# aaakulchyk/replicann

Hardware: AMD Instinct MI355X
Metric: train-step samples/sec (whole node), GPT-2-small DDP at 1/2/4/8 MI355X (higher is better)
Workload: dtype bf16; 1 GPU; model=gpt2-small, global_batch=64, micro_batch_per_gpu=64, seq_len=1024, parallelism=dp1, optimizer=fused AdamW (fp32 master) + grad-norm clip, comm_world=1, gemm_cu_reserve=0

## Files before the change

### csrc/include/gemm_pk.h

```cpp
#pragma once
#include <type_traits>

#include "gemm_impl.h"

namespace rn_gemm_detail {

constexpr int PK_HALF = 16384;
constexpr int PK_RING = 8 * PK_HALF;
constexpr int PK_LDS = PK_RING + 64;
constexpr int PK_CTR_STRIDE = 32;
constexpr int PK_SCHED_INTS = 10 * PK_CTR_STRIDE;

RN_DEV int swz_kcp(int r) { return (((r >> 3) & 3) << 1) | ((r >> 1) & 1); }
RN_DEV int swz_mnp(int k) { return ((k >> 1) & 1) | (((k >> 3) & 1) << 2); }

template <bool KC, bool PERM>
RN_DEV void pk_stage(const u32x4& rs, long ld, int mn_lim, int k_lim, char* lds, int wave, int lane, bool live) {
#pragma unroll
    for (int i = 0; i < 2; ++i) {
        const int ins = wave * 2 + i;
        uint32_t voff;
        if constexpr (KC) {
            const int r = ins * 8 + (lane >> 3);
            const int cg = (lane & 7) ^ (PERM ? swz_kcp(r) : swz_kc(r));
            const int k = cg * 8;
            const bool ok = live && (r < mn_lim) && (k < k_lim);
            voff = ok ? (uint32_t)(((long)r * ld + k) * 2) : 0xFFFFFFF0u;
        } else {
            const int sub = ins >> 3, within = ins & 7;
            const int r = within * 8 + (lane >> 3);
            const int cg = (lane & 7) ^ (PERM ? swz_mnp(r) : swz_mn(r));
            const int mn = sub * 64 + cg * 8;
            const bool ok = live && (r < k_lim) && (mn < mn_lim);
            voff = ok ? (uint32_t)(((long)r * ld + mn) * 2) : 0xFFFFFFF0u;
        }
        dma16(rs, voff, lds + ins * 1024);
    }
}

RN_DEV int swz_f8(int r) { return ((r >> 1) & 3) | (((r >> 4) & 1) << 2); }

RN_DEV s16x8 pk_frag8_mn(const char* lds, int col0, int s, int lane) {
    typedef int i32x2v __attribute__((ext_vector_type(2)));
    const int g = lane >> 4, ii = lane & 15, q = ii >> 1, pp = ii & 1;
    const int cb = col0 + 8 * pp;
    i32x2v v[2];
#pragma unroll
    for (int t = 0; t < 2; ++t) {
        const int row = s * 64 + 16 * g + 8 * t + q;
        const char* a = lds + row * 128 + (((cb >> 4) ^ swz_f8(row)) << 4) + (cb & 15);
        v[t] = __builtin_amdgcn_ds_read_tr8_b64_v2i32((__attribute__((address_space(3))) i32x2v*)a);
    }
    const i32x4 w = {v[0][0], v[0][1], v[1][0], v[1][1]};
    return __builtin_bit_cast(s16x8, w);
}

template <bool KC>
RN_DEV s16x8 pk_frag_a(const char* lds, int mnbase, int s, int lane) {
    return frag<KC>(lds, mnbase, s, lane);
}

template <bool KC>
RN_DEV s16x8 pk_frag_b(const char* lds, int colbase, int j, int s, int lane) {
    if constexpr (KC) {
        const int i = lane & 15;
        const int row = colbase + 8 * (i >> 2) + 4 * j + (i & 3);
        const int chunk = s * 4 + (lane >> 4);
        return *reinterpret_cast<const s16x8*>(lds + row * 128 + ((chunk ^ swz_kcp(row)) << 4));
    } else {
        const char* sub = lds + (colbase >> 6) * 8192;
        const int cl = colbase & 63;
        const int g = lane >> 4, i = lane & 15, q = i >> 2, p = i & 3;
        const int c = (cl >> 3) + p;
        const int half = j ^ (p & 1);
        const int k0 = s * 32 + 8 * g + q;
        const int k1 = k0 + 4;
        const char* a0 = sub + k0 * 128 + ((c ^ swz_mnp(k0)) << 4) + half * 8;
        const char* a1 = sub + k1 * 128 + ((c ^ swz_mnp(k1)) << 4) + half * 8;
        s16x4 v0 = __builtin_amdgcn_ds_read_tr16_b64_v4i16((__attribute__((address_space(3))) s16x4*)a0);
        s16x4 v1 = __builtin_amdgcn_ds_read_tr16_b64_v4i16((__attribute__((address_space(3))) s16x4*)a1);
        s16x8 r;
        r[0] = v0[0]; r[1] = v0[1]; r[2] = v0[2]; r[3] = v0[3];
        r[4] = v1[0]; r[5] = v1[1]; r[6] = v1[2]; r[7] = v1[3];
        return r;
    }
}

RN_DEV __amdgpu_buffer_rsrc_t pk_rsrc(const void* base, uint32_t bytes) {
    const uint64_t bp = (uint64_t)base;
    const uint32_t lo = __builtin_amdgcn_readfirstlane((uint32_t)bp);
    const uint32_t hi = __builtin_amdgcn_readfirstlane((uint32_t)(bp >> 32));
    return __builtin_amdgcn_make_buffer_rsrc((void*)(((uint64_t)hi << 32) | lo), 0, bytes, 0x00020000);
}

RN_DEV u32x4 pk_rsrc_u(const void* base, uint32_t bytes) {
    const uint64_t bp = (uint64_t)base;
    u32x4 r;
    r[0] = __builtin_amdgcn_readfirstlane((uint32_t)bp);
    r[1] = __builtin_amdgcn_readfirstlane((uint32_t)(bp >> 32));
    r[2] = bytes;
    r[3] = 0x00020000u;
    return r;
}

#pragma clang diagnostic push
#pragma clang diagnostic ignored "-Winline-asm"
#if defined(RN_PK_ST_NT)
#define RN_PK_ST_POLICY "nt"
#elif defined(RN_PK_ST_SC)
#define RN_PK_ST_POLICY "sc0 sc1"
#else
#define RN_PK_ST_POLICY ""
#endif
RN_DEV void pk_st16(const u32x4 v, const u32x4& rs, uint32_t voff) {
    asm volatile("buffer_store_dwordx4 %0, %1, %2, 0 offen " RN_PK_ST_POLICY "\n\ts_nop 1" ::"v"(v), "v"(voff), "s"(rs) : "memory");
}
typedef unsigned u32x2v __attribute__((ext_vector_type(2)));
RN_DEV void pk_st8(const u32x2v v, const u32x4& rs, uint32_t voff) {
    asm volatile("buffer_store_dwordx2 %0, %1, %2, 0 offen\n\ts_nop 1" ::"v"(v), "v"(voff), "s"(rs) : "memory");
}
RN_DEV void pk_st16_nt(const u32x4 v, const u32x4& rs, uint32_t voff) {
    asm volatile("buffer_store_dwordx4 %0, %1, %2, 0 offen nt\n\ts_nop 1" ::"v"(v), "v"(voff), "s"(rs) : "memory");
}
#pragma clang diagnostic pop

RN_DEV uint32_t pk_pack2(float a, float b) {
    bf16x2 v = {(bf16)a, (bf16)b};
    return __builtin_bit_cast(uint32_t, v);
}
RN_DEV void pk_unpack8(const u32x4 u, float* f) {
    const uint32_t w[4] = {u.x, u.y, u.z, u.w};
#pragma unroll
    for (int d = 0; d < 4; ++d) {
        f[2 * d] = __builtin_bit_cast(float, w[d] << 16);
        f[2 * d + 1] = __builtin_bit_cast(float, w[d] & 0xFFFF0000u);
    }
}

template <int ACT, bool SPLIT, bool F32>
constexpr int pk_epi_stores() {
    return 16 * ((SPLIT || F32) ? 2 : 1) + (act_fwd(ACT) ? 16 : 0) + (act_bwd(ACT) ? 4 : 0);
}

RN_DEV i32x8 pk_cat8(const s16x8 a, const s16x8 b) {
    const i32x4 x = __builtin_bit_cast(i32x4, a), y = __builtin_bit_cast(i32x4, b);
    return (i32x8){x[0], x[1], x[2], x[3], y[0], y[1], y[2], y[3]};
}

#pragma clang diagnostic push
#pragma clang diagnostic ignored "-Winline-asm"
RN_DEV void pk_deq_issue(uint32_t& v, const int* ctr, bool live) {
    const u32x4 rs = pk_rsrc_u(ctr, ctr ? 4u : 0u);
    const uint32_t off = live ? 0u : 0xFFFFFFF0u;
    v = 1u;
    asm volatile("buffer_atomic_add %0, %1, %2, 0 offen sc0 ; rn_deq_issue" : "+v"(v) : "v"(off), "s"(rs) : "memory");
}
RN_DEV int pk_deq_take(uint32_t v) {
    asm volatile("; rn_deq_take %0" : "+v"(v));
    return (int)__builtin_amdgcn_readfirstlane(v);
}
#pragma clang diagnostic pop

template <bool AK, bool BKC, int ACT, bool SPLIT, bool F32, int DBG = 0, int FP8 = 0, bool DYN = false>
__global__ void __launch_bounds__(512, 1) gemm_pk(GemmArgs p) {
    static_assert(!FP8 || !(DBG & 8), "fp8: no DBG 8");
    static_assert(!FP8 || AK || (!BKC && SPLIT), "fp8 MN-contiguous A: weight gradient (both MN, split-K slabs) only");
    constexpr bool F8A_MN = FP8 && !AK;
    constexpr bool F8B_MN = FP8 && !BKC;
    constexpr bool F8MN = F8A_MN;
    static_assert(!F8B_MN || SPLIT || (ACT == ACT_NONE && !F32), "fp8 MN B, bf16 output: plain epilogue only");
    constexpr int S_EPI = (DBG & 64) ? 0 : pk_epi_stores<ACT, SPLIT, F32>() + ((F8B_MN && !SPLIT) ? 16 : 0);
    static_assert(!DYN || (!FP8 && DBG == 0), "dynamic schedule: bf16 production kernels only");
    constexpr int BM = 256, BN = 256;
    constexpr int WY = 6;
    static_assert(WY + 1 + S_EPI <= 63, "vmcnt range");
    extern __shared__ __attribute__((aligned(16))) char smem[];
    const int lane = threadIdx.x & 63;
    const int wave = __builtin_amdgcn_readfirstlane(threadIdx.x >> 6);
    const int wr = wave >> 2, wc = wave & 3;
    const int G = lane >> 4;
    const int tiles = p.tiles_m * p.tiles_n;
    const int items = tiles * p.split;
    const int grid = gridDim.x;
    const int bid = xcd_remap(blockIdx.x, grid);
    const int nk = p.k_per_split / BK;

    constexpr bool dyn = DYN;
    int* const ring = reinterpret_cast<int*>(smem + PK_RING);
    auto unit_of = [&](int s) -> int {
        if constexpr (!DYN) {
            const int u = bid + s * grid;
            return u < items ? u : -1;
        }
        return __builtin_amdgcn_readfirstlane(*(volatile int*)(ring + (s & 3)));
    };
    auto deq_map = [&](int q, int v) -> int {
        const int per = grid >> 3;
        const bool home = (grid & 7) == 0 && (per & (per - 1)) == 0;
        const int rh = home ? max(0, items / grid - 1) : 0;
        if (q < 8) {
            const int sh = 31 - __builtin_clz(per | 1);
            return (unsigned)v < (unsigned)(rh * per) ? (v >> sh) * grid + q * per + (v & (per - 1)) : -2;
        }
        return (unsigned)v < (unsigned)(items - rh * grid) ? rh * grid + v : -1;
    };

    float alpha = 1.f;
    if (p.alpha) alpha = *p.alpha;
    asm volatile("" ::"v"(alpha));

    auto item_coords = [&](int item, int& m0, int& n0, int& kb, int& ke, int& tm) {
        const int sid = item / tiles;
        int tn;
        group_tile(item - sid * tiles, p.tiles_m, p.tiles_n, tm, tn);
        m0 = tm * BM;
        n0 = tn * BN;
        kb = sid * p.k_per_split;
        ke = min(p.K, kb + p.k_per_split);
    };
    auto lane_mnk = [&](bool isA, int i, int& mn, int& k) {
        const int ins = wave * 2 + i;
        const bool kc = isA ? AK : BKC;
        if (kc) {
            mn = ins * 8 + (lane >> 3);
            k = ((lane & 7) ^ (isA ? swz_kc(mn) : swz_kcp(mn))) * 8;
        } else if (FP8) {
            k = ins * 8 + (lane >> 3);
            mn = ((lane & 7) ^ swz_f8(k)) * 16;
        } else {
            k = (ins & 7) * 8 + (lane >> 3);
            mn = (ins >> 3) * 64 + ((lane & 7) ^ (isA ? swz_mn(k) : swz_mnp(k))) * 8;
        }
    };
    uint32_t a_off[2], b_off[2];
#pragma unroll
    for (int i = 0; i < 2; ++i) {
        int mn, k;
        lane_mnk(true, i, mn, k);
        a_off[i] = (uint32_t)(F8A_MN ? (long)k * p.lda + mn : (AK ? (long)mn * p.lda + k : (long)k * p.lda + mn) * 2);
        lane_mnk(false, i, mn, k);
        b_off[i] = (uint32_t)(F8B_MN ? (long)k * p.ldb + mn : (BKC ? (long)mn * p.ldb + k : (long)k * p.ldb + mn) * 2);
    }
    const long a_step = AK ? (long)BK : (long)BK * p.lda, b_step = BKC ? (long)BK : (long)BK * p.ldb;
    const long a_half = AK ? 128L * p.lda : (F8A_MN ? 64L : 128L), b_half = BKC ? 128L * p.ldb : (F8B_MN ? 64L : 128L);
    const bf16* ca = p.A;
    const bf16* cb = p.B;
    int cml = 0, cnl = 0, ckl = 0, ckt = 0, ct = 0;
    int cu = -1, cs = 0;
    uint32_t intr = 0;
    auto cur_intr = [&]() {
        const bool kf = ckl >= BK;
        intr = kf ? ((cml >= 128 ? 1u : 0u) | (cnl >= 128 ? 2u : 0u) | (cnl >= 256 ? 4u : 0u) | (cml >= 256 ? 8u : 0u))
                  : 0u;
    };
    bool in_loop = false;
    auto cur_set = [&]() {
        int m0, n0, kb, ke, tm;
        item_coords(cu, m0, n0, kb, ke, tm);
        ca = AK ? p.A + (long)m0 * p.lda + kb : p.A + (long)kb * p.lda + (F8A_MN ? m0 / 2 : m0);
        cb = BKC ? p.B + (long)n0 * p.ldb + kb : p.B + (long)kb * p.ldb + (F8B_MN ? n0 / 2 : n0);
        cml = p.M - m0;
        cnl = p.N - n0;
        ckl = ke - kb;
        cur_intr();
    };
    auto cur_adv = [&]() {
        ++ct;
        if (cu < 0) return;
        if (++ckt < nk) {
            ca += a_step;
            cb += b_step;
            ckl -= BK;
            if (ckl < BK) intr = 0u;
            return;
        }
        ckt = 0;
        cu = unit_of(++cs);
        if (cu >= 0) {
            cur_set();
        } else {
            cml = cnl = ckl = 0;
            intr = 0u;
        }
    };
    const uint32_t lds0 = lds_addr(smem) + wave * 2048;
    auto issue_h = [&](auto hc) {
        constexpr int H = decltype(hc)::value;
        if constexpr (DBG & 1) {
            if (in_loop) return;
        }
        const uint32_t dst = lds0 + (uint32_t)(((ct & 1) * 4 + H) * PK_HALF);
        const bool isA = (H == 0 || H == 3);
        const bf16* base = isA ? (H == 3 ? ca + a_half : ca) : (H == 2 ? cb + b_half : cb);
        const int mnl = isA ? (H == 3 ? cml - 128 : cml) : (H == 2 ? cnl - 128 : cnl);
        const u32x4 rs = rsrc_sgpr(base);
        if constexpr (DBG & 16) {
            if (in_loop) {
#pragma unroll
                for (int i = 0; i < 2; ++i) dma16_at(rs, 0xFFFFFFF0u, dst + i * 1024);
                return;
            }
        }
        if (intr & (1u << H)) {
#pragma unroll
            for (int i = 0; i < 2; ++i) dma16_at(rs, isA ? a_off[i] : b_off[i], dst + i * 1024);
        } else {
#pragma unroll
            for (int i = 0; i < 2; ++i) {
                int mn, kk;
                lane_mnk(isA, i, mn, kk);
                const uint32_t o = isA ? a_off[i] : b_off[i];
                const bool f8mn = isA ? F8A_MN : F8B_MN;
                const bool kin = f8mn ? kk < 2 * ckl : kk < ckl;
                dma16_at(rs, (mn < mnl && kin) ? o : 0xFFFFFFF0u, dst + i * 1024);
            }
        }
    };
    using H0 = std::integral_constant<int, 0>;
    using H1 = std::integral_constant<int, 1>;
    using H2 = std::integral_constant<int, 2>;
    using H3 = std::integral_constant<int, 3>;

    f32x4 acc[2][2][4][2];
#pragma unroll
    for (int a = 0; a < 2; ++a)
#pragma unroll
        for (int b = 0; b < 2; ++b)
#pragma unroll
            for (int i = 0; i < 4; ++i)
#pragma unroll
                for (int j = 0; j < 2; ++j) acc[a][b][i][j] = (f32x4){0.f, 0.f, 0.f, 0.f};
    s16x8 Af[4][2], Bl[2][2], Br[2][2];
    auto frag_a = [&](const char* half, int mnbase, int s) -> s16x8 {
        if constexpr (F8A_MN) return pk_frag8_mn(half, mnbase, s, lane);
        else return pk_frag_a<AK>(half, mnbase, s, lane);
    };
    auto frag_b = [&](const char* half, int j, int s) -> s16x8 {
        if constexpr (F8B_MN) return pk_frag8_mn(half, wc * 32 + 16 * j, s, lane);
        else return pk_frag_b<BKC>(half, wc * 32, j, s, lane);
    };

    auto epilogue = [&](int m0, int n0, int tm, int sid) {
        const int mlim = p.M - m0, nlim = p.N - n0;
        const long ldc = SPLIT ? (long)p.N : p.ldc;
        constexpr int ES = (SPLIT || F32) ? 4 : 2;
        char* cbase = SPLIT ? (char*)(p.ws + ((long)sid * p.M + m0) * p.N + n0) : (char*)p.C + ((long)m0 * ldc + n0) * ES;
        const __amdgpu_buffer_rsrc_t crs = pk_rsrc(cbase, 0x7FFFFFF0u);
        const u32x4 crs_u = pk_rsrc_u(cbase, 0x7FFFFFF0u);
        auto off = [&](int mh, int i, int nh, int es, int dc = 0) -> uint32_t {
            const int r = mh * 128 + wr * 64 + i * 16 + (lane & 15);
            const int c = nh * 128 + wc * 32 + (F8B_MN ? 4 : 8) * G + dc;
            return (r < mlim && c < nlim) ? (uint32_t)(((long)r * ldc + c) * es) : 0xFFFFFFF0u;
        };
        float bias[2][8];
#pragma unroll
        for (int nh = 0; nh < 2; ++nh)
#pragma unroll
            for (int t = 0; t < 8; ++t) bias[nh][t] = 0.f;
        if (!SPLIT && !act_bwd(ACT) && p.bias) {
#pragma unroll
            for (int nh = 0; nh < 2; ++nh) {
                const int cb = n0 + nh * 128 + wc * 32;
                if (cb + 32 <= p.N) {
                    const __attribute__((address_space(4))) u32x4* bp =
                        (const __attribute__((address_space(4))) u32x4*)(p.bias + cb);
                    u32x4 b0 = bp[0], b1 = bp[1], b2 = bp[2], b3 = bp[3];
                    asm volatile("" : "+s"(b0), "+s"(b1), "+s"(b2), "+s"(b3));
                    const u32x4 bsel = G == 0 ? b0 : (G == 1 ? b1 : (G == 2 ? b2 : b3));
                    pk_unpack8(bsel, bias[nh]);
                } else if (cb + 8 * G < p.N) {
                    const u32x4 u = *reinterpret_cast<const u32x4*>(p.bias + cb + 8 * G);
                    pk_unpack8(u, bias[nh]);
                }
            }
        }
        const bf16* auxp = SPLIT ? nullptr
                                 : (act_bwd(ACT) ? p.pre : (p.res ? p.res : ((p.accumulate && !F32) ? (const bf16*)p.C : nullptr)));
        constexpr bool AUX2 = act_bwd(ACT) && !SPLIT && !F32;
        u32x4 aux[AUX2 ? 2 : 1][4][2];
        const __amdgpu_buffer_rsrc_t ars = pk_rsrc(auxp ? auxp + (long)m0 * p.ldc + n0 : nullptr, 0x7FFFFFF0u);
        const u32x4 prs = pk_rsrc_u(act_fwd(ACT) && p.pre ? (void*)(p.pre + (long)m0 * p.ldc + n0) : nullptr,
                                    act_fwd(ACT) && p.pre ? 0x7FFFFFF0u : 0u);
        float csum[2][8];
#pragma unroll
        for (int nh = 0; nh < 2; ++nh)
#pragma unroll
            for (int t = 0; t < 8; ++t) csum[nh][t] = 0.f;
#pragma unroll
        for (int mh = 0; mh < 2; ++mh) {
            if (auxp && (!AUX2 || mh == 0)) {
#pragma unroll
                for (int ah = 0; ah < (AUX2 ? 2 : 1); ++ah)
#pragma unroll
                for (int i = 0; i < 4; ++i)
#pragma unroll
                    for (int nh = 0; nh < 2; ++nh) {
#ifdef RN_PK_NO_AUX
                        aux[ah][i][nh] = (u32x4){0x3F803F80u, 0x3F803F80u, 0x3F803F80u, 0x3F803F80u};
#else
                        aux[ah][i][nh] = __builtin_amdgcn_raw_buffer_load_b128(ars, off(AUX2 ? ah : mh, i, nh, 2), 0, 0);
#endif
                    }
#ifndef RN_PK_NO_AUX
                __builtin_amdgcn_s_waitcnt(0x0F70);
#endif
            }
#pragma unroll
            for (int i = 0; i < 4; ++i)
#pragma unroll
                for (int nh = 0; nh < 2; ++nh) {
                    float v[8];
                    const bool swp = !BKC && !F8B_MN && (G & 1);
#pragma unroll
                    for (int c = 0; c < 8; ++c) {
                        const float x0 = acc[mh][nh][i][c >> 2][c & 3], x1 = acc[mh][nh][i][(c >> 2) ^ 1][c & 3];
                        v[c] = (swp ? x1 : x0) * alpha;
                    }
                    if constexpr (SPLIT) {
                        const uint32_t o = off(mh, i, nh, 4);
                        const uint32_t o2 = F8B_MN ? off(mh, i, nh, 4, 16) : (o == 0xFFFFFFF0u ? o : o + 16);
                        pk_st16((u32x4){__builtin_bit_cast(uint32_t, v[0]), __builtin_bit_cast(uint32_t, v[1]),
                                    __builtin_bit_cast(uint32_t, v[2]), __builtin_bit_cast(uint32_t, v[3])},
                            crs_u, o);
                        pk_st16((u32x4){__builtin_bit_cast(uint32_t, v[4]), __builtin_bit_cast(uint32_t, v[5]),
                                    __builtin_bit_cast(uint32_t, v[6]), __builtin_bit_cast(uint32_t, v[7])},
                            crs_u, o2);
                        continue;
                    }
#pragma unroll
                    for (int c = 0; c < 8; ++c) v[c] += bias[nh][c];
                    if constexpr (act_fwd(ACT)) {
                        const u32x4 pu = {pk_pack2(v[0], v[1]), pk_pack2(v[2], v[3]), pk_pack2(v[4], v[5]),
                                          pk_pack2(v[6], v[7])};
                        if constexpr (ACT == ACT_GELU_D) {
                            pk_unpack8(pu, v);
                            float d[8];
#pragma unroll
                            for (int c = 0; c < 8; ++c) v[c] = gelu_and_grad_f(v[c], d[c]);
                            const u32x4 du = {pk_pack2(d[0], d[1]), pk_pack2(d[2], d[3]), pk_pack2(d[4], d[5]),
                                              pk_pack2(d[6], d[7])};
                            pk_st16(du, prs, off(mh, i, nh, 2));
                        } else {
                            pk_st16(pu, prs, off(mh, i, nh, 2));
                            if (p.pre) pk_unpack8(pu, v);
#pragma unroll
                            for (int c = 0; c < 8; ++c) v[c] = act_f<ACT>(v[c]);
                        }
                    }
                    if (auxp) {
                        float ax[8];
                        pk_unpack8(aux[AUX2 ? mh : 0][i][nh], ax);
                        if constexpr (act_bwd(ACT)) {
#pragma unroll
                            for (int c = 0; c < 8; ++c) {
                                v[c] = (float)(bf16)v[c] * act_grad_f<ACT>(ax[c]);
                                csum[nh][c] += (float)(bf16)v[c];
                            }
                        } else {
#pragma unroll
                            for (int c = 0; c < 8; ++c) v[c] += ax[c];
                        }
                    }
                    const uint32_t o = off(mh, i, nh, ES);
                    if constexpr (F32) {
                        float c8[8] = {0.f, 0.f, 0.f, 0.f, 0.f, 0.f, 0.f, 0.f};
                        if (p.accumulate) {
                            const u32x4 c0 = __builtin_amdgcn_raw_buffer_load_b128(crs, o, 0, 0);
                            const u32x4 c1 = __builtin_amdgcn_raw_buffer_load_b128(crs, o == 0xFFFFFFF0u ? o : o + 16, 0, 0);
                            const uint32_t w[8] = {c0.x, c0.y, c0.z, c0.w, c1.x, c1.y, c1.z, c1.w};
#pragma unroll
                            for (int d = 0; d < 8; ++d) c8[d] = __builtin_bit_cast(float, w[d]);
                        }
#pragma unroll
                        for (int c = 0; c < 8; ++c) v[c] += c8[c];
                        pk_st16((u32x4){__builtin_bit_cast(uint32_t, v[0]), __builtin_bit_cast(uint32_t, v[1]),
                                    __builtin_bit_cast(uint32_t, v[2]), __builtin_bit_cast(uint32_t, v[3])},
                            crs_u, o);
                        pk_st16((u32x4){__builtin_bit_cast(uint32_t, v[4]), __builtin_bit_cast(uint32_t, v[5]),
                                    __builtin_bit_cast(uint32_t, v[6]), __builtin_bit_cast(uint32_t, v[7])},
                            crs_u, o == 0xFFFFFFF0u ? o : o + 16);
                    } else {
                        if (p.res && p.accumulate) {
                            float c8[8];
                            pk_unpack8(__builtin_amdgcn_raw_buffer_load_b128(crs, o, 0, 0), c8);
#pragma unroll
                            for (int c = 0; c < 8; ++c) v[c] += c8[c];
                        }
                        const u32x4 ou = {pk_pack2(v[0], v[1]), pk_pack2(v[2], v[3]), pk_pack2(v[4], v[5]),
                                          pk_pack2(v[6], v[7])};
                        if constexpr (DBG & 64) asm volatile("" ::"v"(ou));
                        else if constexpr (F8B_MN) {
                            pk_st8((u32x2v){ou.x, ou.y}, crs_u, o);
                            pk_st8((u32x2v){ou.z, ou.w}, crs_u, off(mh, i, nh, 2, 16));
                        } else if (p.st_nt & 1) pk_st16_nt(ou, crs_u, o);
                        else pk_st16(ou, crs_u, (DBG & 32) ? 0xFFFFFFF0u : o);
                    }
                }
        }
        if constexpr (act_bwd(ACT)) {
#pragma unroll
            for (int nh = 0; nh < 2; ++nh)
#pragma unroll
                for (int c = 0; c < 8; ++c) {
                    float s = csum[nh][c];
                    s += __shfl_xor(s, 1, 64);
                    s += __shfl_xor(s, 2, 64);
                    s += __shfl_xor(s, 4, 64);
                    s += __shfl_xor(s, 8, 64);
                    csum[nh][c] = s;
                }
            float* cpb = p.colpart ? p.colpart + ((long)tm * 2 + wr) * p.N + n0 : nullptr;
            const u32x4 cprs = pk_rsrc_u(cpb, cpb ? 0x7FFFFFF0u : 0u);
#pragma unroll
            for (int nh = 0; nh < 2; ++nh) {
                const int c = nh * 128 + wc * 32 + 8 * G;
                const uint32_t o = ((lane & 15) == 0 && c < nlim) ? (uint32_t)(c * 4) : 0xFFFFFFF0u;
                pk_st16((u32x4){__builtin_bit_cast(uint32_t, csum[nh][0]), __builtin_bit_cast(uint32_t, csum[nh][1]),
                            __builtin_bit_cast(uint32_t, csum[nh][2]), __builtin_bit_cast(uint32_t, csum[nh][3])},
                    cprs, o);
                pk_st16((u32x4){__builtin_bit_cast(uint32_t, csum[nh][4]), __builtin_bit_cast(uint32_t, csum[nh][5]),
                            __builtin_bit_cast(uint32_t, csum[nh][6]), __builtin_bit_cast(uint32_t, csum[nh][7])},
                    cprs, o == 0xFFFFFFF0u ? o : o + 16);
            }
        }
    };

    int deq = blockIdx.x & 7;
    uint32_t deq_v = 0u;

    if constexpr (DYN) {
        if (wave == 0 && lane == 0) {
            int q = blockIdx.x & 7;
            int u = deq_map(q, __hip_atomic_fetch_add(p.sched + q * PK_CTR_STRIDE, 1, __ATOMIC_RELAXED,
                                                      __HIP_MEMORY_SCOPE_AGENT));
            if (u == -2) {
                q = 8;
                u = deq_map(8, __hip_atomic_fetch_add(p.sched + 8 * PK_CTR_STRIDE, 1, __ATOMIC_RELAXED,
                                                      __HIP_MEMORY_SCOPE_AGENT));
            }
            ring[0] = u;
            ring[1] = q | (u < 0 ? 64 : 0);
        }
        __syncthreads();
        deq = __builtin_amdgcn_readfirstlane(ring[1]);
    }
    int c_s = 0;
    int c_u = unit_of(0);
    cu = c_u;
    if (cu >= 0) {
        cur_set();
        issue_h(H0{});
        issue_h(H1{});
        issue_h(H2{});
        issue_h(H3{});
        cur_adv();
        issue_h(H0{});
        issue_h(H1{});
    }
    vm_wait<8>();
    asm volatile("s_barrier" ::: "memory");
    if (wr == 1) asm volatile("s_barrier" ::: "memory");
    in_loop = true;
    __builtin_amdgcn_sched_barrier(0);

    int c_m0 = 0, c_n0 = 0, c_kb = 0, c_ke = 0, c_tm = 0, c_sid = 0, c_kt = 0;
    if (c_u >= 0) {
        item_coords(c_u, c_m0, c_n0, c_kb, c_ke, c_tm);
        c_sid = c_u / tiles;
    }
    int since_epi = 4;

    auto phase_wait = [&](auto xw) {
        if constexpr (DBG & 2) return;
        constexpr bool XW = decltype(xw)::value;
        if (since_epi < 4) {
            if (DYN && XW && wave == 0) vm_wait<WY + 1 + S_EPI>();
            else vm_wait<WY + S_EPI>();
        } else {
            if (DYN && XW && wave == 0) vm_wait<WY + 1>();
            else vm_wait<WY>();
        }
        ++since_epi;
    };
    auto deq_step = [&]() {
        if (DYN && wave == 0) {
            if (deq & 32) {
                const int u = deq_map(deq & 15, pk_deq_take(deq_v));
                if (u == -2) {
                    deq = (deq & 64) | 8 | 16;
                } else {
                    if (lane == 0) *(volatile int*)(ring + ((c_s + 1) & 3)) = u;
                    deq = (deq & ~32) | (u < 0 ? 64 : 0);
                }
            }
            const bool want = (deq & 16) != 0;
            pk_deq_issue(deq_v, p.sched + (deq & 15) * PK_CTR_STRIDE, lane == 0 && want);
            deq = (deq & ~48) | (want ? 32 : 0);
        }
    };
    auto sync_mma_begin = [&]() {
        __builtin_amdgcn_sched_barrier(0);
        asm volatile("s_barrier\n\ts_waitcnt lgkmcnt(0)" ::: "memory");
        __builtin_amdgcn_sched_barrier(0);
        __builtin_amdgcn_s_setprio(1);
    };
    auto sync_mma_end = [&]() {
        __builtin_amdgcn_s_setprio(0);
        __builtin_amdgcn_sched_barrier(0);
        asm volatile("s_barrier" ::: "memory");
        __builtin_amdgcn_sched_barrier(0);
    };
#define RN_PK_MMA(MH, NH, BF)                                                                          \
    if constexpr (FP8) {                                                                               \
        _Pragma("unroll") for (int i_ = 0; i_ < 4; ++i_)                                             \
        _Pragma("unroll") for (int j_ = 0; j_ < 2; ++j_)                                             \
            acc[MH][NH][i_][j_] = __builtin_amdgcn_mfma_scale_f32_16x16x128_f8f6f4(                   \
                pk_cat8(BF[j_][0], BF[j_][1]), pk_cat8(Af[i_][0], Af[i_][1]), acc[MH][NH][i_][j_], 0,     \
                FP8 == 2 ? 1 : 0, 0, 127, 0, 127);                                                     \
    } else {                                                                                           \
    _Pragma("unroll") for (int s_ = 0; s_ < 2; ++s_)                                                 \
    _Pragma("unroll") for (int i_ = 0; i_ < 4; ++i_)                                                 \
    _Pragma("unroll") for (int j_ = 0; j_ < 2; ++j_)                                                 \
        acc[MH][NH][i_][j_] = __builtin_amdgcn_mfma_f32_16x16x32_bf16(BF[j_][s_], Af[i_][s_], acc[MH][NH][i_][j_], 0, 0, 0); \
    }

#define RN_PK_MMA_S(MH, NH, BF, S)                                                                    \
    _Pragma("unroll") for (int i_ = 0; i_ < 4; ++i_)                                                 \
    _Pragma("unroll") for (int j_ = 0; j_ < 2; ++j_)                                                 \
        acc[MH][NH][i_][j_] = __builtin_amdgcn_mfma_f32_16x16x32_bf16(BF[j_][S], Af[i_][S], acc[MH][NH][i_][j_], 0, 0, 0);
#define RN_PK_PHASE(XW, READS, ISSUE, MH, NH, BF)                                                      \
    phase_wait(std::integral_constant<bool, XW>{});                                                    \
    READS                                                                                              \
    if constexpr (!(DBG & 8)) { ISSUE }                                                                \
    sync_mma_begin();                                                                                  \
    if constexpr (DBG & 8) {                                                                           \
        RN_PK_MMA_S(MH, NH, BF, 0)                                                                     \
        __builtin_amdgcn_sched_barrier(0);                                                             \
        ISSUE                                                                                          \
        __builtin_amdgcn_sched_barrier(0);                                                             \
        RN_PK_MMA_S(MH, NH, BF, 1)                                                                     \
    } else {                                                                                           \
        RN_PK_MMA(MH, NH, BF)                                                                          \
    }                                                                                                  \
    sync_mma_end();


    const int n_static = DYN ? 0 : ((items - bid + grid - 1) / grid) * nk;
#pragma unroll 1
    for (int u = 0; DYN ? (c_u >= 0) : (u < n_static); ++u) {
        const char* sl = smem + (u & 1) * (4 * PK_HALF);
        if (dyn && wave == 0 && c_kt == 0 && !(deq & 64)) deq |= 16;
        RN_PK_PHASE(false,
            deq_step();
            _Pragma("unroll") for (int s = 0; s < 2; ++s) {
                _Pragma("unroll") for (int i = 0; i < 4; ++i) Af[i][s] = frag_a(sl, wr * 64 + i * 16, s);
                _Pragma("unroll") for (int j = 0; j < 2; ++j) Bl[j][s] = frag_b(sl + PK_HALF, j, s);
            },
            issue_h(H2{});, 0, 0, Bl)
        RN_PK_PHASE(true,
            _Pragma("unroll") for (int s = 0; s < 2; ++s)
                _Pragma("unroll") for (int j = 0; j < 2; ++j) Br[j][s] = frag_b(sl + 2 * PK_HALF, j, s);,
            issue_h(H3{});, 0, 1, Br)
        RN_PK_PHASE(true,
            _Pragma("unroll") for (int s = 0; s < 2; ++s)
                _Pragma("unroll") for (int i = 0; i < 4; ++i) Af[i][s] = frag_a(sl + 3 * PK_HALF, wr * 64 + i * 16, s);,
            cur_adv(); issue_h(H0{});, 1, 1, Br)
        RN_PK_PHASE(true, , issue_h(H1{});, 1, 0, Bl)
        if (++c_kt == nk) {
            if constexpr (DYN) vm_wait<8>();
            if constexpr (!(DBG & 4)) {
                epilogue(c_m0, c_n0, c_tm, c_sid);
            } else {
#pragma unroll
                for (int a = 0; a < 2; ++a)
#pragma unroll
                    for (int b = 0; b < 2; ++b)
#pragma unroll
                        for (int i = 0; i < 4; ++i)
#pragma unroll
                            for (int j = 0; j < 2; ++j) asm volatile("" : "+v"(acc[a][b][i][j]));
            }
            since_epi = 0;
#pragma unroll
            for (int a = 0; a < 2; ++a)
#pragma unroll
                for (int b = 0; b < 2; ++b)
#pragma unroll
                    for (int i = 0; i < 4; ++i)
#pragma unroll
                        for (int j = 0; j < 2; ++j) acc[a][b][i][j] = (f32x4){0.f, 0.f, 0.f, 0.f};
            c_kt = 0;
            c_u = unit_of(++c_s);
            if (c_u >= 0) {
                item_coords(c_u, c_m0, c_n0, c_kb, c_ke, c_tm);
                c_sid = c_u / tiles;
            }
        }
    }
#undef RN_PK_MMA
#undef RN_PK_MMA_S
#undef RN_PK_PHASE
    if (wr == 0) asm volatile("s_barrier" ::: "memory");
    if (DYN && wave == 0 && lane == 0) {
        int* const cnt = p.sched;
        if (__hip_atomic_fetch_add(cnt + 9 * PK_CTR_STRIDE, 1, __ATOMIC_RELAXED, __HIP_MEMORY_SCOPE_AGENT) == grid - 1) {
#pragma unroll
            for (int i = 0; i < 10; ++i) __hip_atomic_store(cnt + i * PK_CTR_STRIDE, 0, __ATOMIC_RELAXED, __HIP_MEMORY_SCOPE_AGENT);
        }
    }
    (void)c_kb;
    (void)c_ke;
}

}
extern "C" int* rn_gemm_sched_slot(int dev, hipStream_t st);
extern "C" int rn_gemm_get_reserve();
namespace rn_gemm_detail {
inline int rn_gemm_st_nt(const GemmArgs& a) {
    return (a.split <= 1 && (long)a.M * a.N * 2 > (1024L << 20)) ? 1 : 0;
}
}
namespace rn_gemm_detail {

inline int* pk_sched_slot(const GemmArgs& a, hipStream_t st) {
    if (a.k_per_split / BK < 5) return nullptr;
    int dev = 0;
    (void)hipGetDevice(&dev);
    return rn_gemm_sched_slot(dev, st);
}

template <bool AK, bool BKC, int ACT, bool SPLIT, bool F32, int DBG = 0, int FP8 = 0, bool DYN = false>
void launch_pk_t(GemmArgs& a, hipStream_t st) {
    auto kern = gemm_pk<AK, BKC, ACT, SPLIT, F32, DBG, FP8, DYN>;
    static int attr_dev = -1;
    int dev = 0;
    (void)hipGetDevice(&dev);
    if (attr_dev != dev) {
        (void)hipFuncSetAttribute((const void*)kern, hipFuncAttributeMaxDynamicSharedMemorySize, PK_LDS);
        attr_dev = dev;
    }
    const int items = a.tiles_m * a.tiles_n * a.split;
    int cus = 256;
    {
        static int cu_dev = -1, cu_n = 256;
        if (cu_dev != dev) {
            hipDeviceProp_t prop;
            if (hipGetDeviceProperties(&prop, dev) == hipSuccess) cu_n = prop.multiProcessorCount;
            cu_dev = dev;
        }
        cus = cu_n;
    }
    a.st_nt = rn_gemm_st_nt(a);
    const int reserve = rn_gemm_get_reserve();
    if (reserve > 0 && reserve < cus) cus -= reserve;
    if (!DYN) a.sched = nullptr;
    const int grid = items < cus ? items : cus;
    kern<<<grid, 512, PK_LDS, st>>>(a);
}

}
```

Baseline: 1024 samples/s.

## Stream epilogue aux loads through a sliding window with counted vmcnt waits

Replaces the blocking load-all-then-wait of residual/pre-activation aux tiles in the GEMM epilogue with an 8-entry sliding window of inline-asm buffer loads. Each row group waits only for its own loads, using a computed vmcnt that accounts for interleaved stores, and issues the next loads after processing. The aim is to overlap aux global-load latency with epilogue math and stores and to cut aux register pressure. It relies on fragile vmcnt accounting across asm-issued loads and stores, so a wrong count could read stale data.

Measured after the change: 1030 samples/s (median of 6 runs). About the same (+0.6%).

```diff
diff --git a/csrc/include/gemm_pk.h b/csrc/include/gemm_pk.h
--- a/csrc/include/gemm_pk.h
+++ b/csrc/include/gemm_pk.h
@@ -159,7 +159,19 @@
     asm volatile("; rn_deq_take %0" : "+v"(v));
     return (int)__builtin_amdgcn_readfirstlane(v);
 }
+RN_DEV void pk_aux_issue(u32x4& v, const u32x4& rs, uint32_t voff) {
+    asm volatile("buffer_load_dwordx4 %0, %1, %2, 0 offen ; rn_aux_issue" : "=v"(v) : "v"(voff), "s"(rs) : "memory");
+}
+RN_DEV void pk_aux_take(u32x4& v) { asm volatile("; rn_aux_take %0" : "+v"(v)); }
 #pragma clang diagnostic pop
+
+constexpr int PK_WIN = 8;
+constexpr int pk_aux_younger(int R, int S2) {
+    const int t = 2 * R + 1, HR = PK_WIN / 2;
+    int y = t < PK_WIN ? PK_WIN - 1 - t : 0;
+    for (int r = t < PK_WIN ? 0 : R - HR + 1; r < R; ++r) y += S2 + (r + HR < 8 ? 2 : 0);
+    return y < 63 ? y : 63;
+}
 
 template <bool AK, bool BKC, int ACT, bool SPLIT, bool F32, int DBG = 0, int FP8 = 0, bool DYN = false>
 __global__ void __launch_bounds__(512, 1) gemm_pk(GemmArgs p) {
@@ -173,6 +185,7 @@
     static_assert(!DYN || (!FP8 && DBG == 0), "dynamic schedule: bf16 production kernels only");
     constexpr int BM = 256, BN = 256;
     constexpr int WY = 6;
+    constexpr int S_ROW = (DBG & 64) ? 0 : ((SPLIT || F32) ? 2 : 1) + (act_fwd(ACT) ? 1 : 0);
     static_assert(WY + 1 + S_EPI <= 63, "vmcnt range");
     extern __shared__ __attribute__((aligned(16))) char smem[];
     const int lane = threadIdx.x & 63;
@@ -340,7 +353,29 @@
         else return pk_frag_b<BKC>(half, wc * 32, j, s, lane);
     };
 
+    auto tile_off = [&](int mlim, int nlim, long ldc, int mh, int i, int nh, int es, int dc) -> uint32_t {
+        int ln = lane;
+        asm volatile("" : "+v"(ln));
+        const int r = mh * 128 + wr * 64 + i * 16 + (ln & 15);
+        const int c = nh * 128 + wc * 32 + (F8B_MN ? 4 : 8) * (ln >> 4) + dc;
+        return (r < mlim && c < nlim) ? (uint32_t)(((long)r * ldc + c) * es) : 0xFFFFFFF0u;
+    };
+    const bf16* const auxp = (SPLIT || (DBG & 4))
+        ? nullptr
+        : (act_bwd(ACT) ? p.pre : (p.res ? p.res : ((p.accumulate && !F32) ? (const bf16*)p.C : nullptr)));
+    constexpr bool AUX_ASM = !FP8;
+#ifdef RN_PK_NO_AUX
+    const bool aux_ld = false;
+#else
+    const bool aux_ld = AUX_ASM && auxp != nullptr;
+#endif
+    auto aux_issue = [&](u32x4& dst, int e, int m0, int n0) {
+        const u32x4 rs = pk_rsrc_u(auxp + (long)m0 * p.ldc + n0, 0x7FFFFFF0u);
+        pk_aux_issue(dst, rs, tile_off(p.M - m0, p.N - n0, p.ldc, e >> 3, (e >> 1) & 3, e & 1, 2, 0));
+    };
+
     auto epilogue = [&](int m0, int n0, int tm, int sid) {
+        u32x4 aux[PK_WIN];
         const int mlim = p.M - m0, nlim = p.N - n0;
         const long ldc = SPLIT ? (long)p.N : p.ldc;
         constexpr int ES = (SPLIT || F32) ? 4 : 2;
@@ -348,10 +383,12 @@
         const __amdgpu_buffer_rsrc_t crs = pk_rsrc(cbase, 0x7FFFFFF0u);
         const u32x4 crs_u = pk_rsrc_u(cbase, 0x7FFFFFF0u);
         auto off = [&](int mh, int i, int nh, int es, int dc = 0) -> uint32_t {
-            const int r = mh * 128 + wr * 64 + i * 16 + (lane & 15);
-            const int c = nh * 128 + wc * 32 + (F8B_MN ? 4 : 8) * G + dc;
-            return (r < mlim && c < nlim) ? (uint32_t)(((long)r * ldc + c) * es) : 0xFFFFFFF0u;
+            return tile_off(mlim, nlim, ldc, mh, i, nh, es, dc);
         };
+        if (aux_ld) {
+#pragma unroll
+            for (int e = 0; e < PK_WIN; ++e) aux_issue(aux[e], e, m0, n0);
+        }
         float bias[2][8];
 #pragma unroll
         for (int nh = 0; nh < 2; ++nh)
@@ -374,11 +411,6 @@
                 }
             }
         }
-        const bf16* auxp = SPLIT ? nullptr
-                                 : (act_bwd(ACT) ? p.pre : (p.res ? p.res : ((p.accumulate && !F32) ? (const bf16*)p.C : nullptr)));
-        constexpr bool AUX2 = act_bwd(ACT) && !SPLIT && !F32;
-        u32x4 aux[AUX2 ? 2 : 1][4][2];
-        const __amdgpu_buffer_rsrc_t ars = pk_rsrc(auxp ? auxp + (long)m0 * p.ldc + n0 : nullptr, 0x7FFFFFF0u);
         const u32x4 prs = pk_rsrc_u(act_fwd(ACT) && p.pre ? (void*)(p.pre + (long)m0 * p.ldc + n0) : nullptr,
                                     act_fwd(ACT) && p.pre ? 0x7FFFFFF0u : 0u);
         float csum[2][8];
@@ -386,27 +418,41 @@
         for (int nh = 0; nh < 2; ++nh)
 #pragma unroll
             for (int t = 0; t < 8; ++t) csum[nh][t] = 0.f;
+        auto aux_wait = [&](auto rc) {
+            constexpr int R = decltype(rc)::value;
+            vm_wait<pk_aux_younger(R, 2 * S_ROW)>();
+        };
 #pragma unroll
         for (int mh = 0; mh < 2; ++mh) {
-            if (auxp && (!AUX2 || mh == 0)) {
-#pragma unroll
-                for (int ah = 0; ah < (AUX2 ? 2 : 1); ++ah)
-#pragma unroll
-                for (int i = 0; i < 4; ++i)
-#pragma unroll
-                    for (int nh = 0; nh < 2; ++nh) {
+#pragma unroll
+            for (int i = 0; i < 4; ++i) {
+                if (aux_ld) {
+                    switch (4 * mh + i) {
+                        case 0: aux_wait(std::integral_constant<int, 0>{}); break;
+                        case 1: aux_wait(std::integral_constant<int, 1>{}); break;
+                        case 2: aux_wait(std::integral_constant<int, 2>{}); break;
+                        case 3: aux_wait(std::integral_constant<int, 3>{}); break;
+                        case 4: aux_wait(std::integral_constant<int, 4>{}); break;
+                        case 5: aux_wait(std::integral_constant<int, 5>{}); break;
+                        case 6: aux_wait(std::integral_constant<int, 6>{}); break;
+                        default: aux_wait(std::integral_constant<int, 7>{}); break;
+                    }
+                    pk_aux_take(aux[(8 * mh + 2 * i) % PK_WIN]);
+                    pk_aux_take(aux[(8 * mh + 2 * i + 1) % PK_WIN]);
+                } else if (auxp) {
 #ifdef RN_PK_NO_AUX
-                        aux[ah][i][nh] = (u32x4){0x3F803F80u, 0x3F803F80u, 0x3F803F80u, 0x3F803F80u};
+                    aux[(8 * mh + 2 * i) % PK_WIN] = aux[(8 * mh + 2 * i + 1) % PK_WIN] =
+                        (u32x4){0x3F803F80u, 0x3F803F80u, 0x3F803F80u, 0x3F803F80u};
 #else
-                        aux[ah][i][nh] = __builtin_amdgcn_raw_buffer_load_b128(ars, off(AUX2 ? ah : mh, i, nh, 2), 0, 0);
+                    if (i == 0) {
+                        const __amdgpu_buffer_rsrc_t ars = pk_rsrc(auxp + (long)m0 * p.ldc + n0, 0x7FFFFFF0u);
+#pragma unroll
+                        for (int e = 0; e < 8; ++e)
+                            aux[e] = __builtin_amdgcn_raw_buffer_load_b128(ars, off(mh, e >> 1, e & 1, 2), 0, 0);
+                        __builtin_amdgcn_s_waitcnt(0x0F70);
+                    }
 #endif
-                    }
-#ifndef RN_PK_NO_AUX
-                __builtin_amdgcn_s_waitcnt(0x0F70);
-#endif
-            }
-#pragma unroll
-            for (int i = 0; i < 4; ++i)
+                }
 #pragma unroll
                 for (int nh = 0; nh < 2; ++nh) {
                     float v[8];
@@ -449,7 +495,7 @@
                     }
                     if (auxp) {
                         float ax[8];
-                        pk_unpack8(aux[AUX2 ? mh : 0][i][nh], ax);
+                        pk_unpack8(aux[(8 * mh + 2 * i + nh) % PK_WIN], ax);
                         if constexpr (act_bwd(ACT)) {
 #pragma unroll
                             for (int c = 0; c < 8; ++c) {
@@ -496,6 +542,14 @@
                         else pk_st16(ou, crs_u, (DBG & 32) ? 0xFFFFFFF0u : o);
                     }
                 }
+                if (aux_ld && 8 * mh + 2 * i + PK_WIN < 16) {
+#pragma unroll
+                    for (int nh = 0; nh < 2; ++nh) {
+                        const int e = 8 * mh + 2 * i + nh + PK_WIN;
+                        aux_issue(aux[e % PK_WIN], e, m0, n0);
+                    }
+                }
+            }
         }
         if constexpr (act_bwd(ACT)) {
 #pragma unroll
```
